# teticio/audio-diffusion

Hardware: NVIDIA H100
Metric: mel-spectrograms/sec (1000-step DDPM, 256x256x1) (higher is better)
Workload: dtype bf16 operands, fp32 accumulate (fp32 master weights, fp64 GroupNorm sums)

## Files before the change

audio_diffusion_b200/_lib.py:

```python
from __future__ import annotations

import ctypes as C
import os

_HERE = os.path.dirname(os.path.abspath(__file__))
LIB_PATH = os.environ.get("B200AD_LIB") or os.path.join(_HERE, "libb200ad.so")

MAX_BLOCKS = 8


class UNetConfigC(C.Structure):
    _fields_ = [
        ("in_channels", C.c_int), ("out_channels", C.c_int), ("layers_per_block", C.c_int), ("num_blocks", C.c_int),
        ("block_out_channels", C.c_int * MAX_BLOCKS), ("down_attn", C.c_int * MAX_BLOCKS),
        ("up_attn", C.c_int * MAX_BLOCKS), ("norm_num_groups", C.c_int), ("norm_eps", C.c_float),
        ("attention_head_dim", C.c_int), ("cross_attention_dim", C.c_int), ("down_cross", C.c_int * MAX_BLOCKS),
        ("up_cross", C.c_int * MAX_BLOCKS),
    ]


class VAEConfigC(C.Structure):
    _fields_ = [
        ("in_channels", C.c_int), ("out_channels", C.c_int), ("latent_channels", C.c_int), ("layers_per_block", C.c_int),
        ("num_blocks", C.c_int), ("block_out_channels", C.c_int * MAX_BLOCKS), ("norm_num_groups", C.c_int),
# ... 26 lines not shown
    "b200ad_unet_param_name": (C.c_char_p, [_VP, _I]),
    "b200ad_unet_param_shape": (_I, [_VP, _I, C.POINTER(C.c_int64)]),
    "b200ad_unet_packed_bytes": (_SZ, [_VP]),
    "b200ad_unet_workspace_bytes": (_SZ, [_VP, _I, _I, _I]),
    "b200ad_unet_set_params": (_I, [_VP, C.POINTER(_VP), _VP, _SZ, _VP]),
    "b200ad_unet_bind_workspace": (_I, [_VP, _VP, _SZ, _I, _I, _I, _VP]),
    "b200ad_unet_forward": (_I, [_VP, _VP, _VP, _VP, _VP]),
    "b200ad_unet_set_encoding": (_I, [_VP, _VP, _I]),
    "b200ad_unet_forward_step": (_I, [_VP, _VP, _VP, _VP, C.POINTER(StepCoefC), _VP, _VP, _VP]),
    "b200ad_unet_forward_step_dev": (_I, [_VP, _VP, _VP, _VP, _VP, _VP, _VP]),
    "b200ad_step_scalars_upload": (_I, [C.POINTER(StepCoefC), C.c_float, _VP, _VP, C.c_int, _VP]),
    "b200ad_unet_profile_step": (_I, [_VP, _VP, _VP, _VP, C.POINTER(StepCoefC), _VP, C.POINTER(C.c_float),
                                      C.POINTER(_I), C.POINTER(C.c_double), _I, _VP]),
    "b200ad_unet_debug_tensor": (_I, [_VP, C.c_char_p, _VP, C.POINTER(_I), _VP]),
    "b200ad_unet_last_launch_count": (_I, [_VP]),
    "b200ad_unet_set_training": (_I, [_VP, _I]),
    "b200ad_unet_grad_floats": (_SZ, [_VP]),
    "b200ad_unet_grad_offset": (_SZ, [_VP, _I]),
    "b200ad_unet_backward_bytes": (_SZ, [_VP]),
    "b200ad_unet_bind_backward": (_I, [_VP, _VP, _SZ, _VP, _VP]),
    "b200ad_unet_backward": (_I, [_VP, _VP, _VP, _I, _VP]),
    "b200ad_unet_backward_launch_count": (_I, [_VP]),
    "b200ad_vae_set_training": (_I, [_VP, _I]),
    "b200ad_vae_grad_floats": (_SZ, [_VP]),
    "b200ad_vae_grad_offset": (_SZ, [_VP, _I]),
    "b200ad_vae_backward_bytes": (_SZ, [_VP]),
    "b200ad_vae_bind_backward": (_I, [_VP, _VP, _SZ, _VP, _VP]),
    "b200ad_vae_decoder_backward": (_I, [_VP, _VP, _VP, _I, _VP]),
    "b200ad_vae_encoder_backward": (_I, [_VP, _VP, _VP, _I, _VP]),
    "b200ad_vae_backward_launch_count": (_I, [_VP]),
# ... 74 lines not shown
```

audio_diffusion_b200/csrc/common.cuh:

```cuda
#pragma once
#include <cuda_bf16.h>
#include <cuda_runtime.h>
#include <stdint.h>
#include <stdio.h>

namespace b200ad {

typedef double stat_t;

struct Geom {
  int N, H, W, Wp, lead, PL;
};
__host__ __device__ inline Geom make_geom(int N, int H, int W) {
  Geom g;
  g.N = N; g.H = H; g.W = W; g.Wp = W + 1; g.lead = g.Wp + 8;
  g.PL = g.lead + H * g.Wp + g.Wp + 8 + 512;
  return g;
}

#ifdef __CUDACC__
__device__ __forceinline__ uint32_t smem_u32(const void* p) {
  return static_cast<uint32_t>(__cvta_generic_to_shared(p));
}
__device__ __forceinline__ void mbar_init(uint32_t bar, uint32_t count) {
// ... 49 lines not shown
__device__ __forceinline__ void bulk_wait_read_all() { asm volatile("cp.async.bulk.wait_group.read 0;" ::: "memory"); }
__device__ __forceinline__ void bulk_wait_all() { asm volatile("cp.async.bulk.wait_group 0;" ::: "memory"); }
__device__ __forceinline__ void named_bar_sync(int id, int nthreads) {
  asm volatile("bar.sync %0, %1;" ::"r"(id), "r"(nthreads) : "memory");
}

__device__ __forceinline__ void tensor_g2s_5d(uint32_t dst_smem, const void* tmap, int c0, int c1, int c2, int c3, int c4,
                                              uint32_t bar) {
  asm volatile(
      "cp.async.bulk.tensor.5d.shared::cluster.global.tile.mbarrier::complete_tx::bytes [%0], [%1, {%2, %3, %4, %5, %6}], [%7];"
      ::"r"(dst_smem), "l"(tmap), "r"(c0), "r"(c1), "r"(c2), "r"(c3), "r"(c4), "r"(bar) : "memory");
}
__device__ __forceinline__ void tensor_s2g_5d(const void* tmap, int c0, int c1, int c2, int c3, int c4, uint32_t src_smem) {
  asm volatile("cp.async.bulk.tensor.5d.global.shared::cta.tile.bulk_group [%0, {%1, %2, %3, %4, %5}], [%6];"
               ::"l"(tmap), "r"(c0), "r"(c1), "r"(c2), "r"(c3), "r"(c4), "r"(src_smem) : "memory");
}

__device__ __forceinline__ void bulk_prefetch_l2(const void* src, uint32_t bytes) {
  asm volatile("cp.async.bulk.prefetch.L2.global [%0], %1;" ::"l"(src), "r"(bytes) : "memory");
}

__device__ __forceinline__ uint64_t gmma_desc(uint32_t saddr, uint32_t lbo_bytes, uint32_t sbo_bytes) {
  uint64_t d = 0;
  d |= (uint64_t)((saddr >> 4) & 0x3FFF);
  d |= (uint64_t)((lbo_bytes >> 4) & 0x3FFF) << 16;
  d |= (uint64_t)((sbo_bytes >> 4) & 0x3FFF) << 32;
  return d;
}
__device__ __forceinline__ void wgmma_fence() { asm volatile("wgmma.fence.sync.aligned;" ::: "memory"); }
__device__ __forceinline__ void wgmma_commit() { asm volatile("wgmma.commit_group.sync.aligned;" ::: "memory"); }
// ... 65 lines not shown
        "+f"(d[24]), "+f"(d[25]), "+f"(d[26]), "+f"(d[27]), "+f"(d[28]), "+f"(d[29]), "+f"(d[30]), "+f"(d[31]),
        "+f"(d[32]), "+f"(d[33]), "+f"(d[34]), "+f"(d[35]), "+f"(d[36]), "+f"(d[37]), "+f"(d[38]), "+f"(d[39]),
        "+f"(d[40]), "+f"(d[41]), "+f"(d[42]), "+f"(d[43]), "+f"(d[44]), "+f"(d[45]), "+f"(d[46]), "+f"(d[47]),
        "+f"(d[48]), "+f"(d[49]), "+f"(d[50]), "+f"(d[51]), "+f"(d[52]), "+f"(d[53]), "+f"(d[54]), "+f"(d[55]),
        "+f"(d[56]), "+f"(d[57]), "+f"(d[58]), "+f"(d[59]), "+f"(d[60]), "+f"(d[61]), "+f"(d[62]), "+f"(d[63]),
        "+f"(d[64]), "+f"(d[65]), "+f"(d[66]), "+f"(d[67]), "+f"(d[68]), "+f"(d[69]), "+f"(d[70]), "+f"(d[71]),
        "+f"(d[72]), "+f"(d[73]), "+f"(d[74]), "+f"(d[75]), "+f"(d[76]), "+f"(d[77]), "+f"(d[78]), "+f"(d[79]),
        "+f"(d[80]), "+f"(d[81]), "+f"(d[82]), "+f"(d[83]), "+f"(d[84]), "+f"(d[85]), "+f"(d[86]), "+f"(d[87]),
        "+f"(d[88]), "+f"(d[89]), "+f"(d[90]), "+f"(d[91]), "+f"(d[92]), "+f"(d[93]), "+f"(d[94]), "+f"(d[95]),
        "+f"(d[96]), "+f"(d[97]), "+f"(d[98]), "+f"(d[99]), "+f"(d[100]), "+f"(d[101]), "+f"(d[102]), "+f"(d[103]),
        "+f"(d[104]), "+f"(d[105]), "+f"(d[106]), "+f"(d[107]), "+f"(d[108]), "+f"(d[109]), "+f"(d[110]), "+f"(d[111]),
        "+f"(d[112]), "+f"(d[113]), "+f"(d[114]), "+f"(d[115]), "+f"(d[116]), "+f"(d[117]), "+f"(d[118]), "+f"(d[119]),
        "+f"(d[120]), "+f"(d[121]), "+f"(d[122]), "+f"(d[123]), "+f"(d[124]), "+f"(d[125]), "+f"(d[126]), "+f"(d[127])
      : "l"(a), "l"(b), "r"(1), "n"(TA), "n"(TB));
}

__device__ __forceinline__ bool elect_one() {
  uint32_t pred;
  asm volatile(
      "{\n\t.reg .pred p;\n\t"
      "elect.sync _|p, 0xffffffff;\n\t"
      "selp.u32 %0, 1, 0, p;\n\t}"
      : "=r"(pred));
  return pred != 0;
}

__device__ __forceinline__ void fence_proxy_async_smem() { asm volatile("fence.proxy.async.shared::cta;" ::: "memory"); }

__device__ __forceinline__ float tanh_approx(float x) {
  float y;
// ... 48 lines not shown
```

audio_diffusion_b200/csrc/conv_tc.cu:

```cuda
#include <cuda.h>
#include <cudaTypedefs.h>

#include <cstdlib>

#include "conv_tc.cuh"

namespace b200ad {

struct alignas(64) ConvMaps {
  CUtensorMap src[CONV_MAXSEG];
  CUtensorMap out;
};

__host__ __device__ __forceinline__ int window_pixels(const ConvParams& p, const ConvSeg& sg, int G) {
  return p.tile2d ? (CONV_TW + sg.hl + sg.hr) * (CONV_TH + sg.ht + sg.hb)
                  : G * CONV_TM + (sg.ht + sg.hb) * p.Wp + sg.hl + sg.hr;
}
__host__ __device__ __forceinline__ int window_pitch(const ConvParams& p, const ConvSeg& sg) {
  return p.tile2d ? CONV_TW + sg.hl + sg.hr : p.Wp;
}

constexpr int CONV_THREADS = 384;
constexpr int CONV_XF_THREADS = 64;
constexpr int CONV_SPLANE = CONV_MAXG * CONV_TM * 16;
constexpr int CONV_STG_WG = 8 * CONV_SPLANE;
constexpr int CONV_STAGING = 2 * CONV_STG_WG;

struct WorkItem {
  int n, ntile, m0, G;
  int r0, c0;
};

__device__ __forceinline__ WorkItem decode_work(const ConvParams& p, int w) {
  WorkItem wi;
  wi.ntile = w % p.ntiles_n;
  const int gidx = w / p.ntiles_n;
  if (p.tile2d) {
    wi.n = gidx / p.groups_per_img;
    const int t = gidx - wi.n * p.groups_per_img, tx = t / p.tiles_y;
    wi.r0 = (t - tx * p.tiles_y) * CONV_TH;
    wi.c0 = tx * CONV_TW;
    wi.m0 = 0;
    wi.G = CONV_MAXG;
    return wi;
  }
  wi.r0 = wi.c0 = 0;
  if (p.pack) {
    wi.n = gidx * p.pack;
    wi.m0 = 0;
    wi.G = min(p.pack, p.N - wi.n);
    return wi;
  }
  wi.n = gidx / p.groups_per_img;
  const int g = gidx - wi.n * p.groups_per_img;
  wi.m0 = g * (CONV_MAXG * CONV_TM);
  const int rem = p.H * p.Wp - wi.m0;
// ... 4 lines not shown
template <bool SILU>
__device__ __forceinline__ uint4 xform_vec(uint4 v, const f32x2_t (&sc)[4], const f32x2_t (&sh)[4]) {
  uint32_t u[4] = {v.x, v.y, v.z, v.w};
#pragma unroll
  for (int e = 0; e < 4; ++e) {
    f32x2_t a = f2_fma(f2_from_bf16x2(u[e]), sc[e], sh[e]);
    if (SILU) {
      const float2 f = f2_unpack(a);
      a = f2_fma(a, f2_pack(tanh_approx(f.x), tanh_approx(f.y)), a);
    }
    u[e] = f2_to_bf16x2(a);
  }
  return make_uint4(u[0], u[1], u[2], u[3]);
}

__global__ void __launch_bounds__(CONV_THREADS, 1) conv_tc_kernel(const __grid_constant__ ConvParams p,
                                                                  const __grid_constant__ ConvMaps maps) {
  constexpr int ASM = CONV_AS_MAX, BSM = CONV_BS_MAX;
  const int AS = p.as;
  const int BS = p.bs;
  extern __shared__ __align__(128) uint8_t smem[];
  const int warp = __shfl_sync(0xffffffffu, (int)(threadIdx.x >> 5), 0);
  const int lane = threadIdx.x & 31;
  const int a_bytes = p.a_stage;

  uint8_t* bring = smem + AS * a_bytes;
  uint8_t* stg = bring + BS * CONV_B_SLOT;
  uint8_t* ctrl = stg + CONV_STAGING;
  uint64_t* bars = reinterpret_cast<uint64_t*>(ctrl);
  const uint32_t smem_base = smem_u32(smem);
// ... 28 lines not shown
    for (int w = blockIdx.x; w < p.total_work; w += gridDim.x) {
      const WorkItem wi = decode_work(p, w);
      for (int s = 0; s < p.nseg; ++s) {
        const ConvSeg& sg = p.seg[s];
        const uint32_t row_bytes = (uint32_t)window_pixels(p, sg, wi.G) * 16u;
        for (int ks = 0; ks < sg.ksteps; ++ks) {
          const uint32_t full = bar_fullA + 8 * stage;
          if (lane == 0) {
            mbar_wait(bar_emptyA + 8 * stage, phase ^ 1);
            mbar_arrive_expect_tx(full, 2u * row_bytes);
          }
          __syncwarp();
          const long long plane = (long long)(2 * ks + (lane & 1)) * p.PL;
          if (p.tile2d) {
            if (lane == 0)
              tensor_g2s_5d(smem_base + stage * a_bytes, &maps.src[s], 0, wi.c0 - sg.hl, wi.r0 - sg.ht, 2 * ks, wi.n, full);
          } else if (!p.pack) {
            const int pix0 = p.lead + wi.m0 - sg.ht * p.Wp - sg.hl;
            if (lane < 2)
              bulk_g2s(smem_base + stage * a_bytes + (uint32_t)lane * row_bytes,
                       sg.src + (long long)wi.n * sg.img_stride + (plane + pix0) * 8, row_bytes, full);
          } else {
            const int g = lane >> 1, lead_px = sg.ht * p.Wp + sg.hl, trail_px = sg.hb * p.Wp + sg.hr;
            const int cnt = CONV_TM + (g == 0 ? lead_px : 0) + (g == wi.G - 1 ? trail_px : 0);
            const int doff = (g == 0) ? 0 : lead_px + g * CONV_TM;
            const int pix0 = p.lead - (g == 0 ? lead_px : 0);
            if (g < wi.G && lane < 2 * CONV_MAXG)
              bulk_g2s(smem_base + stage * a_bytes + (uint32_t)(lane & 1) * row_bytes + (uint32_t)doff * 16u,
                       sg.src + (long long)(wi.n + g) * sg.img_stride + (plane + pix0) * 8, (uint32_t)cnt * 16u, full);
          }
          if (++stage == AS) { stage = 0; phase ^= 1; }
// ... 53 lines not shown
      for (int s = 0, ks = 0; s < p.nseg;) {
        const ConvSeg& sg = p.seg[s];
        const uint32_t xlbo = (uint32_t)window_pixels(p, sg, wi.G) * 16u;
        const uint32_t xsbo = p.tile2d ? (uint32_t)window_pitch(p, sg) * 16u : 128u;
        const int ntaps = sg.ntaps;
        mbar_wait(bar_readyA + 8 * sa, pa);
        const uint32_t abase = smem_base + sa * a_bytes;
        for (int t0 = 0; t0 < ntaps; t0 += CONV_BT) {
          mbar_wait(bar_fullB + 8 * sb, pb);
          const uint32_t bbase = bring_base + sb * CONV_B_SLOT + (uint32_t)(cw * 1024);
          const int nt = min(CONV_BT, ntaps - t0);
          wgmma_fence();
          for (int t = 0; t < nt; ++t) {
            const uint64_t wdesc = gmma_desc(bbase + (uint32_t)t * CONV_B_TAP, (CONV_NT / 8) * 128, 128);
            const uint64_t xdesc = gmma_desc(abase + (uint32_t)sg.aoff[t0 + t] * 16u, xlbo, xsbo);
            if (wi.G == 2) wgmma_m64n256k16<0, 0>(acc, wdesc, xdesc);
            else           wgmma_m64n128k16<0, 0>(acc, wdesc, xdesc);
          }
          wgmma_commit();
          wgmma_wait<1>();
          release();
          pend_b = sb;
          pend_a = (t0 + CONV_BT >= ntaps) ? sa : -1;
          if (++sb == BS) { sb = 0; pb ^= 1; }
        }
        if (++sa == AS) { sa = 0; pa ^= 1; }
        if (++ks == sg.ksteps) { ks = 0; ++s; }
      }
      wgmma_wait<0>();
      release();

      if (issuer) bulk_wait_read_all();
// ... 48 lines not shown
                  const int c = wi.ntile * CONV_NT + cw * 64 + wq * 16 + 8 * h + (lane >> 2);
                  stat_t* sdst = p.stats + ((long long)n * (p.cout >> 2) + (c >> 2)) * 2;
                  atomicAdd(sdst, (stat_t)s1);
                  atomicAdd(sdst + 1, (stat_t)s2);
                }
                ssum[h] = 0.f;
                ssq[h] = 0.f;
              }
            }
          }
        }
      }
      if (p.tile2d) {
        fence_proxy_async_smem();
        named_bar_sync(1 + cw, 128);
        if (tid == 0 && !(p.dbg & 2)) {
          tensor_s2g_5d(&maps.out, 0, wi.c0, wi.r0, wi.ntile * 16 + cw * 8, wi.n, stg_w);
          bulk_commit();
        }
      } else if (!p.up2) {
        fence_proxy_async_smem();
        named_bar_sync(1 + cw, 128);
        const int g = tid >> 3, pl = tid & 7;
        if (issuer && g < wi.G && !(p.dbg & 2)) {
          const int n = p.pack ? wi.n + g : wi.n;
          bulk_s2g(p.out + (long long)n * out_img_stride + (long long)(wi.ntile * 16 + cw * 8 + pl) * og.PL * 8 +
                       (long long)(p.lead + (p.pack ? 0 : wi.m0 + CONV_TM * g)) * 8,
                   stg_w + (uint32_t)(pl * CONV_SPLANE + g * CONV_TM * 16), (uint32_t)CONV_TM * 16u);
          bulk_commit();
        }
      } else {
        named_bar_sync(1 + cw, 128);
// ... 151 lines not shown
        int n = i / Ct, c = i - n * Ct;
        for (; i < total; i += CONV_THREADS) {
          const int gi = n * f.groups + (int)(((float)c + 0.5f) * inv_cpg);
          const float sc = __ldg(f.gamma + c) * grstd[gi];
          f.ss[i] = make_float2(sc, __ldg(f.beta + c) - gmean[gi] * sc);
          n += dn;
          c += dc;
          if (c >= Ct) { c -= Ct; ++n; }
        }
      }
      if (threadIdx.x == 0) *f.counter = 0u;
    }
  }
}

static cudaError_t encode_pf8_map(CUtensorMap* m, const __nv_bfloat16* base, const ConvParams& p, int planes,
                                  long long img_stride, int bw, int bh, int bplanes) {
  static PFN_cuTensorMapEncodeTiled_v12000 encode = nullptr;
  if (!encode) {
    void* fn = nullptr;
    cudaDriverEntryPointQueryResult q;
    cudaError_t e = cudaGetDriverEntryPointByVersion("cuTensorMapEncodeTiled", &fn, 12000, cudaEnableDefault, &q);
    if (e != cudaSuccess) return e;
    if (q != cudaDriverEntryPointSuccess || !fn) return cudaErrorNotSupported;
    encode = reinterpret_cast<PFN_cuTensorMapEncodeTiled_v12000>(fn);
  }
  const cuuint64_t dim[5] = {8, (cuuint64_t)p.W, (cuuint64_t)p.H, (cuuint64_t)planes, (cuuint64_t)p.N};
  const cuuint64_t stride[4] = {16, (cuuint64_t)p.Wp * 16, (cuuint64_t)p.PL * 16, (cuuint64_t)img_stride * 2};
  const cuuint32_t box[5] = {8, (cuuint32_t)bw, (cuuint32_t)bh, (cuuint32_t)bplanes, 1};
  const cuuint32_t estride[5] = {1, 1, 1, 1, 1};
  const CUresult r = encode(m, CU_TENSOR_MAP_DATA_TYPE_BFLOAT16, 5, (void*)(base + (long long)p.lead * 8), dim, stride, box,
                            estride, CU_TENSOR_MAP_INTERLEAVE_NONE, CU_TENSOR_MAP_SWIZZLE_NONE, CU_TENSOR_MAP_L2_PROMOTION_L2_256B,
                            CU_TENSOR_MAP_FLOAT_OOB_FILL_NONE);
  return r == CUDA_SUCCESS ? cudaSuccess : cudaErrorInvalidValue;
}

cudaError_t launch_conv_tc(const ConvParams& p_in, int num_sms, cudaStream_t stream) {
  const char* dbg_env = getenv("B200AD_CONV_DBG");
  const int dbg = dbg_env ? atoi(dbg_env) : 0;
  if (p_in.nseg < 1 || p_in.nseg > CONV_MAXSEG) return cudaErrorInvalidValue;
  ConvParams p = p_in;
  p.dbg = dbg;
  for (int s = 0; s < p.nseg; ++s) {
    ConvSeg& sg = p.seg[s];
    if (sg.ntaps > CONV_MAXTAPS || sg.ksteps < 1) return cudaErrorInvalidValue;
    if (sg.wtile_stride == 0) sg.wtile_stride = (long long)sg.ksteps * sg.ntaps * (CONV_B_TAP / 2);
    sg.ht = sg.hb = sg.hl = sg.hr = 0;
    for (int t = 0; t < sg.ntaps; ++t) {
      sg.ht |= sg.dh[t] < 0; sg.hb |= sg.dh[t] > 0;
      sg.hl |= sg.dw[t] < 0; sg.hr |= sg.dw[t] > 0;
    }
  }
  p.groups_per_img = (p.H * p.Wp + CONV_MAXG * CONV_TM - 1) / (CONV_MAXG * CONV_TM);
  p.ntiles_n = p.cout / CONV_NT;
  p.total_work = p.N * p.groups_per_img * p.ntiles_n;
  p.pack = 0;
  int fits = 1;
  for (int s = 0; s < p.nseg; ++s) {
    const ConvSeg& sg = p.seg[s];
    if (p.H * p.Wp + sg.hb * p.Wp + sg.hr > CONV_TM || sg.ht * p.Wp + sg.hl > CONV_TM) fits = 0;
  }
  if (fits) {
    int best = 1;
    long long best_cost = -1;
    for (int g = 1; g <= CONV_MAXG; g *= 2) {
      const long long items = (long long)((p.N + g - 1) / g) * p.ntiles_n;
      const long long cost = ((items + num_sms - 1) / num_sms) * g;
      if (best_cost < 0 || cost <= best_cost) { best_cost = cost; best = g; }
    }
    p.pack = best;
    p.total_work = ((p.N + best - 1) / best) * p.ntiles_n;
  }
  const int tiles_img = (p.H * p.Wp + CONV_TM - 1) / CONV_TM;
  const int max_g = p.pack ? p.pack : (tiles_img < CONV_MAXG ? tiles_img : CONV_MAXG);
  p.tile2d = 0;
  if (!p.pack && !p.up2 && !(dbg & 4096) && p.W % CONV_TW == 0 && p.H % CONV_TH == 0) {
    ConvParams q = p;
    q.tile2d = 1;
    long long flat = 0, tiled = 0;
    for (int s = 0; s < p.nseg; ++s) {
      flat += window_pixels(p, p.seg[s], max_g);
      tiled += window_pixels(q, p.seg[s], max_g);
    }
    if (tiled < flat) {
      p.tile2d = 1;
      p.tiles_y = p.H / CONV_TH;
      p.groups_per_img = (p.W / CONV_TW) * p.tiles_y;
      p.total_work = p.N * p.groups_per_img * p.ntiles_n;
    }
  }
  int a_stage = 0;
  for (int s = 0; s < p.nseg; ++s) {
    const ConvSeg& sg = p.seg[s];
    const int npix = window_pixels(p, sg, max_g), pitch = window_pitch(p, sg);
    a_stage = npix * 32 > a_stage ? npix * 32 : a_stage;
    if (sg.ntaps > CONV_MAXTAPS || sg.ntaps > CONV_BT * (CONV_BS - 1) || npix > 0x3FFF) return cudaErrorInvalidValue;
    for (int t = 0; t < sg.ntaps; ++t) p.seg[s].aoff[t] = (sg.dh[t] + sg.ht) * pitch + sg.dw[t] + sg.hl;
  }
  p.a_stage = (a_stage + 255) & ~255;
  ConvMaps maps{};
  if (p.tile2d) {
    for (int s = 0; s < p.nseg; ++s) {
      const ConvSeg& sg = p.seg[s];
      cudaError_t e = encode_pf8_map(&maps.src[s], sg.src, p, 2 * sg.ksteps, sg.img_stride, CONV_TW + sg.hl + sg.hr,
                                     CONV_TH + sg.ht + sg.hb, 2);
      if (e != cudaSuccess) return e;
    }
    cudaError_t e = encode_pf8_map(&maps.out, p.out, p, p.cout / 8, (long long)(p.cout / 8) * p.PL * 8, CONV_TW, CONV_TH, 8);
    if (e != cudaSuccess) return e;
  }
  p.as = CONV_AS;
  p.bs = CONV_BS;
  auto rings_fit = [&](int as, int bs) {
    return (size_t)as * p.a_stage + (size_t)bs * CONV_B_SLOT + CONV_STAGING + 2048 <= (size_t)CONV_SMEM_MAX;
  };
  while (p.as < 6 && rings_fit(p.as + 1, p.bs)) ++p.as;
  while (p.bs < CONV_BS_MAX && rings_fit(p.as, p.bs + 1)) ++p.bs;
  while (p.as < CONV_AS_MAX && rings_fit(p.as + 1, p.bs)) ++p.as;
  const size_t smem = (size_t)p.as * p.a_stage + (size_t)p.bs * CONV_B_SLOT + CONV_STAGING + 1024;
  if (smem > (size_t)CONV_SMEM_MAX) return cudaErrorInvalidValue;
  const int grid = p.total_work < num_sms ? p.total_work : num_sms;
  if (grid <= 0) return cudaSuccess;
  static size_t attr = 0;
  if (smem > attr) {
    cudaError_t e = cudaFuncSetAttribute(conv_tc_kernel, cudaFuncAttributeMaxDynamicSharedMemorySize, (int)smem);
    if (e != cudaSuccess) return e;
    attr = smem;
  }
  cudaLaunchConfig_t cfg = {};
  cfg.gridDim = dim3((unsigned)grid);
  cfg.blockDim = dim3(CONV_THREADS);
  cfg.dynamicSmemBytes = smem;
  cfg.stream = stream;
  cudaLaunchAttribute at[1];
  at[0].id = cudaLaunchAttributeProgrammaticStreamSerialization;
  at[0].val.programmaticStreamSerializationAllowed = 1;
  cfg.attrs = at;
  cfg.numAttrs = 1;
  return cudaLaunchKernelEx(&cfg, conv_tc_kernel, p, maps);
}

__global__ void pack_identity_kernel(int channels, __nv_bfloat16* __restrict__ dst, long long nvec) {
  const long long id = (long long)blockIdx.x * blockDim.x + threadIdx.x;
  if (id >= nvec) return;
  const int r = (int)(id & 7), n8 = (int)((id >> 3) & 15), k8 = (int)((id >> 7) & 1);
  const long long rest = id >> 8;
  const int ksteps = channels / 16;
  const int ks = (int)(rest % ksteps), ntile = (int)(rest / ksteps);
  const int co = ntile * 128 + n8 * 8 + r;
  const int ci0 = ks * 16 + k8 * 8;
  uint32_t o[4];
#pragma unroll
  for (int e = 0; e < 4; ++e) o[e] = pack_bf16x2(co == ci0 + 2 * e ? 1.f : 0.f, co == ci0 + 2 * e + 1 ? 1.f : 0.f);
  reinterpret_cast<uint4*>(dst)[id] = make_uint4(o[0], o[1], o[2], o[3]);
// ... 9 lines not shown
```

audio_diffusion_b200/csrc/conv_tc.cuh:

```cuda
#pragma once
#include "common.cuh"

namespace b200ad {

constexpr int CONV_NT = 128;
constexpr int CONV_TM = 128;
constexpr int CONV_MAXG = 2;
constexpr int CONV_TW = 8;
constexpr int CONV_TH = CONV_MAXG * CONV_TM / CONV_TW;
constexpr int CONV_MAXSEG = 4;
constexpr int CONV_MAXTAPS = 9;
constexpr int CONV_B_TAP = 16 * CONV_NT * 2;
constexpr int CONV_SMEM_MAX = 227 * 1024;

constexpr int CONV_BT = 3;
constexpr int CONV_B_SLOT = CONV_BT * CONV_B_TAP;
constexpr int CONV_AS_MAX = 8;
constexpr int CONV_AS = 3;
constexpr int CONV_BS = 5;
constexpr int CONV_BS_MAX = 10;

struct ConvSeg {
  const __nv_bfloat16* src;
  const __nv_bfloat16* wpack;
// ... 15 lines not shown
  int C[2];
  const float* gamma;
  const float* beta;
  float2* ss;
  unsigned* counter;
  int groups, HW;
  float eps;
};

struct ConvParams {
  ConvSeg seg[CONV_MAXSEG];
  int nseg;
  int N, H, W, Wp, lead, PL;
  int a_stage;
  int tile2d;
  int tiles_y;
  int groups_per_img;
  int ntiles_n;
  int total_work;
  int pack;
  int as, bs;
  int cout;
  __nv_bfloat16* out;
  const float* bias;
  const float* temb;
  int temb_stride;
  stat_t* stats;
  int up2, oy, ox;
  ConvGnFin fin;
  int dbg;
};

cudaError_t launch_conv_tc(const ConvParams& p, int num_sms, cudaStream_t stream);

cudaError_t launch_pack_identity(int channels, __nv_bfloat16* dst, cudaStream_t s);

}
```

audio_diffusion_b200/csrc/unet.cu:

```cuda
#include "unet.cuh"

namespace b200ad {

thread_local char g_err[512] = "";
int set_err(const char* fmt, ...) {
  va_list ap;
  va_start(ap, fmt);
  vsnprintf(g_err, sizeof(g_err), fmt, ap);
  va_end(ap);
  return -1;
}

}

using namespace b200ad;


namespace b200ad {

static std::vector<Block> unet_blocks(const b200ad_unet_config& c) {
  const int nb = c.num_blocks, D = c.block_out_channels[0] * 4, X = c.cross_attention_dim;
  const int* boc = c.block_out_channels;
  std::vector<Block> bl;
  add_block(bl, BK_UNET_HEAD, "", c.in_channels, boc[0], "").temb = D;
// ... 192 lines not shown
      double k = 0;
      for (int s = 0; s < p.nseg; ++s) {
        bool ident = false;
        for (const auto& kv : h->ident_off)
          if ((const uint8_t*)p.seg[s].wpack == h->packed + kv.second) ident = true;
        if (!ident) k += (double)(p.up2 ? 9 : p.seg[s].ntaps) * p.seg[s].ksteps * 16;
      }
      fl = 2.0 * p.N * p.H * p.W * p.cout * k;
    }
    op_flops[i] = fl;
  }
  for (auto& e : ev) cudaEventDestroy(e);
  return nops;
}

extern "C" int b200ad_unet_set_encoding(b200ad_unet* h, const float* enc, int S) {
  if (!h->cfg.cross_attention_dim) return set_err("set_encoding: this U-Net is unconditional");
  if (S < 1) return set_err("set_encoding: empty encoder sequence");
  h->enc = enc;
  h->enc_S = S;
  return 0;
}

extern "C" int b200ad_unet_forward(b200ad_unet* h, const float* x, const float* t, float* eps_out, void* stream) {
  RunArgs a;
  a.in = x; a.t = t; a.out = eps_out;
  return run_plan(h, a, (cudaStream_t)stream);
}
extern "C" int b200ad_unet_forward_step(b200ad_unet* h, const float* x, const float* t, const float* z,
                                        const b200ad_step_coef* coef, float* x_out, float* eps_out, void* stream) {
// ... 30 lines not shown
```

include/b200ad.h:

```cpp
#ifndef B200AD_H
#define B200AD_H
#include <stddef.h>
#include <stdint.h>

#ifdef __cplusplus
extern "C" {
#endif

#define B200AD_MAX_BLOCKS 8

const char* b200ad_last_error(void);
int b200ad_version(void);

typedef struct {
  int in_channels, out_channels;
  int layers_per_block;
  int num_blocks;
  int block_out_channels[B200AD_MAX_BLOCKS];
  int down_attn[B200AD_MAX_BLOCKS];
  int up_attn[B200AD_MAX_BLOCKS];
  int norm_num_groups;
  float norm_eps;
  int attention_head_dim;
  int cross_attention_dim;
// ... 29 lines not shown
int b200ad_unet_forward_step(b200ad_unet* h, const float* x, const float* t, const float* z,
                             const b200ad_step_coef* coef, float* x_out, float* eps_out, void* stream);

int b200ad_unet_forward_step_dev(b200ad_unet* h, const float* x, const float* t, const float* z,
                                 const b200ad_step_coef* coef_dev, float* x_out, void* stream);
int b200ad_step_scalars_upload(const b200ad_step_coef* coef, float t, b200ad_step_coef* coef_dev, float* t_dev, int n,
                               void* stream);

int b200ad_unet_debug_tensor(b200ad_unet* h, const char* name, float* dst, int* dims, void* stream);

int b200ad_unet_profile_step(b200ad_unet* h, const float* x, const float* t, const float* z,
                             const b200ad_step_coef* coef, float* x_out, float* op_ms, int* op_kind,
                             double* op_flops, int max_ops, void* stream);

int b200ad_unet_last_launch_count(const b200ad_unet* h);

int b200ad_unet_set_training(b200ad_unet* h, int on);
size_t b200ad_unet_grad_floats(b200ad_unet* h);
size_t b200ad_unet_grad_offset(b200ad_unet* h, int i);
size_t b200ad_unet_backward_bytes(b200ad_unet* h);
int b200ad_unet_bind_backward(b200ad_unet* h, void* arena, size_t bytes, float* grads, void* stream);
int b200ad_unet_backward(b200ad_unet* h, const float* x, const float* g_eps, int accumulate, void* stream);
int b200ad_unet_backward_launch_count(const b200ad_unet* h);

typedef struct {
  int in_channels, out_channels;
  int latent_channels;
  int layers_per_block;
  int num_blocks;
  int block_out_channels[B200AD_MAX_BLOCKS];
// ... 86 lines not shown
```

Baseline: 0.8489.

## Add 16x16 square 2D conv tiles with cost-based tile shape selection

Generalizes the 2D-tiled implicit-GEMM conv from a fixed 8x32 window to selectable 8x32 or 16x16 tiles. A planner scores each shape by padded work, item count and halo-window pixels per k-step. A templated SQUARE kernel path issues paired m64n128 wgmma instructions and per-row TMA stores, and the TMA maps move to a 4D layout. Square tiles are also enabled for upsample-fused convs, which reduces halo reloads but adds more store instructions and more planner complexity; a plan-inspection API is exported as well.

```diff
diff --git a/audio_diffusion_b200/_lib.py b/audio_diffusion_b200/_lib.py
--- a/audio_diffusion_b200/_lib.py
+++ b/audio_diffusion_b200/_lib.py
@@ -64,6 +64,7 @@
                                       C.POINTER(_I), C.POINTER(C.c_double), _I, _VP]),
     "b200ad_unet_debug_tensor": (_I, [_VP, C.c_char_p, _VP, C.POINTER(_I), _VP]),
     "b200ad_unet_last_launch_count": (_I, [_VP]),
+    "b200ad_unet_conv_plan": (_I, [_VP, _I, _I, _I, _I, C.POINTER(_I), _I]),
     "b200ad_unet_set_training": (_I, [_VP, _I]),
     "b200ad_unet_grad_floats": (_SZ, [_VP]),
     "b200ad_unet_grad_offset": (_SZ, [_VP, _I]),
diff --git a/audio_diffusion_b200/csrc/common.cuh b/audio_diffusion_b200/csrc/common.cuh
--- a/audio_diffusion_b200/csrc/common.cuh
+++ b/audio_diffusion_b200/csrc/common.cuh
@@ -87,6 +87,16 @@
 __device__ __forceinline__ void tensor_s2g_5d(const void* tmap, int c0, int c1, int c2, int c3, int c4, uint32_t src_smem) {
   asm volatile("cp.async.bulk.tensor.5d.global.shared::cta.tile.bulk_group [%0, {%1, %2, %3, %4, %5}], [%6];"
                ::"l"(tmap), "r"(c0), "r"(c1), "r"(c2), "r"(c3), "r"(c4), "r"(src_smem) : "memory");
+}
+
+__device__ __forceinline__ void tensor_g2s_4d(uint32_t dst_smem, const void* tmap, int c0, int c1, int c2, int c3, uint32_t bar) {
+  asm volatile(
+      "cp.async.bulk.tensor.4d.shared::cluster.global.tile.mbarrier::complete_tx::bytes [%0], [%1, {%2, %3, %4, %5}], [%6];"
+      ::"r"(dst_smem), "l"(tmap), "r"(c0), "r"(c1), "r"(c2), "r"(c3), "r"(bar) : "memory");
+}
+__device__ __forceinline__ void tensor_s2g_4d(const void* tmap, int c0, int c1, int c2, int c3, uint32_t src_smem) {
+  asm volatile("cp.async.bulk.tensor.4d.global.shared::cta.tile.bulk_group [%0, {%1, %2, %3, %4}], [%5];"
+               ::"l"(tmap), "r"(c0), "r"(c1), "r"(c2), "r"(c3), "r"(src_smem) : "memory");
 }
 
 __device__ __forceinline__ void bulk_prefetch_l2(const void* src, uint32_t bytes) {
@@ -182,6 +192,39 @@
         "+f"(d[120]), "+f"(d[121]), "+f"(d[122]), "+f"(d[123]), "+f"(d[124]), "+f"(d[125]), "+f"(d[126]), "+f"(d[127])
       : "l"(a), "l"(b), "r"(1), "n"(TA), "n"(TB));
 }
+__device__ __forceinline__ void wgmma_m64n128k16_x2(float* d, uint64_t a, uint64_t b0, uint64_t b1) {
+  asm volatile(
+      "{\n\t.reg .pred p;\n\tsetp.ne.b32 p, %131, 0;\n\t"
+      "wgmma.mma_async.sync.aligned.m64n128k16.f32.bf16.bf16 {"
+      "%0, %1, %2, %3, %4, %5, %6, %7, %8, %9, %10, %11, %12, %13, %14, %15, "
+      "%16, %17, %18, %19, %20, %21, %22, %23, %24, %25, %26, %27, %28, %29, %30, %31, "
+      "%32, %33, %34, %35, %36, %37, %38, %39, %40, %41, %42, %43, %44, %45, %46, %47, "
+      "%48, %49, %50, %51, %52, %53, %54, %55, %56, %57, %58, %59, %60, %61, %62, %63"
+      "}, %128, %129, p, 1, 1, 0, 0;\n\t"
+      "wgmma.mma_async.sync.aligned.m64n128k16.f32.bf16.bf16 {"
+      "%64, %65, %66, %67, %68, %69, %70, %71, %72, %73, %74, %75, %76, %77, %78, %79, "
+      "%80, %81, %82, %83, %84, %85, %86, %87, %88, %89, %90, %91, %92, %93, %94, %95, "
+      "%96, %97, %98, %99, %100, %101, %102, %103, %104, %105, %106, %107, %108, %109, %110, %111, "
+      "%112, %113, %114, %115, %116, %117, %118, %119, %120, %121, %122, %123, %124, %125, %126, %127"
+      "}, %128, %130, p, 1, 1, 0, 0;\n\t}"
+      : "+f"(d[0]), "+f"(d[1]), "+f"(d[2]), "+f"(d[3]), "+f"(d[4]), "+f"(d[5]), "+f"(d[6]), "+f"(d[7]),
+        "+f"(d[8]), "+f"(d[9]), "+f"(d[10]), "+f"(d[11]), "+f"(d[12]), "+f"(d[13]), "+f"(d[14]), "+f"(d[15]),
+        "+f"(d[16]), "+f"(d[17]), "+f"(d[18]), "+f"(d[19]), "+f"(d[20]), "+f"(d[21]), "+f"(d[22]), "+f"(d[23]),
+        "+f"(d[24]), "+f"(d[25]), "+f"(d[26]), "+f"(d[27]), "+f"(d[28]), "+f"(d[29]), "+f"(d[30]), "+f"(d[31]),
+        "+f"(d[32]), "+f"(d[33]), "+f"(d[34]), "+f"(d[35]), "+f"(d[36]), "+f"(d[37]), "+f"(d[38]), "+f"(d[39]),
+        "+f"(d[40]), "+f"(d[41]), "+f"(d[42]), "+f"(d[43]), "+f"(d[44]), "+f"(d[45]), "+f"(d[46]), "+f"(d[47]),
+        "+f"(d[48]), "+f"(d[49]), "+f"(d[50]), "+f"(d[51]), "+f"(d[52]), "+f"(d[53]), "+f"(d[54]), "+f"(d[55]),
+        "+f"(d[56]), "+f"(d[57]), "+f"(d[58]), "+f"(d[59]), "+f"(d[60]), "+f"(d[61]), "+f"(d[62]), "+f"(d[63]),
+        "+f"(d[64]), "+f"(d[65]), "+f"(d[66]), "+f"(d[67]), "+f"(d[68]), "+f"(d[69]), "+f"(d[70]), "+f"(d[71]),
+        "+f"(d[72]), "+f"(d[73]), "+f"(d[74]), "+f"(d[75]), "+f"(d[76]), "+f"(d[77]), "+f"(d[78]), "+f"(d[79]),
+        "+f"(d[80]), "+f"(d[81]), "+f"(d[82]), "+f"(d[83]), "+f"(d[84]), "+f"(d[85]), "+f"(d[86]), "+f"(d[87]),
+        "+f"(d[88]), "+f"(d[89]), "+f"(d[90]), "+f"(d[91]), "+f"(d[92]), "+f"(d[93]), "+f"(d[94]), "+f"(d[95]),
+        "+f"(d[96]), "+f"(d[97]), "+f"(d[98]), "+f"(d[99]), "+f"(d[100]), "+f"(d[101]), "+f"(d[102]), "+f"(d[103]),
+        "+f"(d[104]), "+f"(d[105]), "+f"(d[106]), "+f"(d[107]), "+f"(d[108]), "+f"(d[109]), "+f"(d[110]), "+f"(d[111]),
+        "+f"(d[112]), "+f"(d[113]), "+f"(d[114]), "+f"(d[115]), "+f"(d[116]), "+f"(d[117]), "+f"(d[118]), "+f"(d[119]),
+        "+f"(d[120]), "+f"(d[121]), "+f"(d[122]), "+f"(d[123]), "+f"(d[124]), "+f"(d[125]), "+f"(d[126]), "+f"(d[127])
+      : "l"(a), "l"(b0), "l"(b1), "r"(1));
+}
 
 __device__ __forceinline__ bool elect_one() {
   uint32_t pred;
diff --git a/audio_diffusion_b200/csrc/conv_tc.cu b/audio_diffusion_b200/csrc/conv_tc.cu
--- a/audio_diffusion_b200/csrc/conv_tc.cu
+++ b/audio_diffusion_b200/csrc/conv_tc.cu
@@ -13,11 +13,11 @@
 };
 
 __host__ __device__ __forceinline__ int window_pixels(const ConvParams& p, const ConvSeg& sg, int G) {
-  return p.tile2d ? (CONV_TW + sg.hl + sg.hr) * (CONV_TH + sg.ht + sg.hb)
+  return p.tile2d ? (p.tw + sg.hl + sg.hr) * (p.th + sg.ht + sg.hb)
                   : G * CONV_TM + (sg.ht + sg.hb) * p.Wp + sg.hl + sg.hr;
 }
 __host__ __device__ __forceinline__ int window_pitch(const ConvParams& p, const ConvSeg& sg) {
-  return p.tile2d ? CONV_TW + sg.hl + sg.hr : p.Wp;
+  return p.tile2d ? p.tw + sg.hl + sg.hr : p.Wp;
 }
 
 constexpr int CONV_THREADS = 384;
@@ -25,6 +25,9 @@
 constexpr int CONV_SPLANE = CONV_MAXG * CONV_TM * 16;
 constexpr int CONV_STG_WG = 8 * CONV_SPLANE;
 constexpr int CONV_STAGING = 2 * CONV_STG_WG;
+static size_t conv_smem_bytes(const ConvParams& p) {
+  return (size_t)p.as * p.a_stage + (size_t)p.bs * CONV_B_SLOT + CONV_STAGING + 1024;
+}
 
 struct WorkItem {
   int n, ntile, m0, G;
@@ -38,8 +41,8 @@
   if (p.tile2d) {
     wi.n = gidx / p.groups_per_img;
     const int t = gidx - wi.n * p.groups_per_img, tx = t / p.tiles_y;
-    wi.r0 = (t - tx * p.tiles_y) * CONV_TH;
-    wi.c0 = tx * CONV_TW;
+    wi.r0 = (t - tx * p.tiles_y) * p.th;
+    wi.c0 = tx * p.tw;
     wi.m0 = 0;
     wi.G = CONV_MAXG;
     return wi;
@@ -74,6 +77,7 @@
   return make_uint4(u[0], u[1], u[2], u[3]);
 }
 
+template <bool SQUARE>
 __global__ void __launch_bounds__(CONV_THREADS, 1) conv_tc_kernel(const __grid_constant__ ConvParams p,
                                                                   const __grid_constant__ ConvMaps maps) {
   constexpr int ASM = CONV_AS_MAX, BSM = CONV_BS_MAX;
@@ -132,7 +136,7 @@
           const long long plane = (long long)(2 * ks + (lane & 1)) * p.PL;
           if (p.tile2d) {
             if (lane == 0)
-              tensor_g2s_5d(smem_base + stage * a_bytes, &maps.src[s], 0, wi.c0 - sg.hl, wi.r0 - sg.ht, 2 * ks, wi.n, full);
+              tensor_g2s_4d(smem_base + stage * a_bytes, &maps.src[s], 8 * (wi.c0 - sg.hl), wi.r0 - sg.ht, 2 * ks, wi.n, full);
           } else if (!p.pack) {
             const int pix0 = p.lead + wi.m0 - sg.ht * p.Wp - sg.hl;
             if (lane < 2)
@@ -216,8 +220,13 @@
           for (int t = 0; t < nt; ++t) {
             const uint64_t wdesc = gmma_desc(bbase + (uint32_t)t * CONV_B_TAP, (CONV_NT / 8) * 128, 128);
             const uint64_t xdesc = gmma_desc(abase + (uint32_t)sg.aoff[t0 + t] * 16u, xlbo, xsbo);
-            if (wi.G == 2) wgmma_m64n256k16<0, 0>(acc, wdesc, xdesc);
-            else           wgmma_m64n128k16<0, 0>(acc, wdesc, xdesc);
+            if constexpr (SQUARE) {
+              wgmma_m64n128k16_x2(acc, wdesc, xdesc, xdesc + (128u >> 4));
+            } else if (wi.G == 2) {
+              wgmma_m64n256k16<0, 0>(acc, wdesc, xdesc);
+            } else {
+              wgmma_m64n128k16<0, 0>(acc, wdesc, xdesc);
+            }
           }
           wgmma_commit();
           wgmma_wait<1>();
@@ -296,8 +305,17 @@
       if (p.tile2d) {
         fence_proxy_async_smem();
         named_bar_sync(1 + cw, 128);
-        if (tid == 0 && !(p.dbg & 2)) {
-          tensor_s2g_5d(&maps.out, 0, wi.c0, wi.r0, wi.ntile * 16 + cw * 8, wi.n, stg_w);
+        if (SQUARE) {
+          const int g = tid >> 3, pl = tid & 7;
+          if (issuer && !(p.dbg & 2)) {
+            const uint32_t src = stg_w + (uint32_t)(pl * CONV_SPLANE + g * CONV_TM * 16);
+            const int c = wi.c0 + 8 * g, plane = wi.ntile * 16 + cw * 8 + pl;
+            if (p.up2) tensor_s2g_5d(&maps.out, 0, c, wi.r0, plane, wi.n, src);
+            else       tensor_s2g_4d(&maps.out, 8 * c, wi.r0, plane, wi.n, src);
+            bulk_commit();
+          }
+        } else if (tid == 0 && !(p.dbg & 2)) {
+          tensor_s2g_4d(&maps.out, 8 * wi.c0, wi.r0, wi.ntile * 16 + cw * 8, wi.n, stg_w);
           bulk_commit();
         }
       } else if (!p.up2) {
@@ -479,8 +497,8 @@
   }
 }
 
-static cudaError_t encode_pf8_map(CUtensorMap* m, const __nv_bfloat16* base, const ConvParams& p, int planes,
-                                  long long img_stride, int bw, int bh, int bplanes) {
+static cudaError_t encode_pf8_map(CUtensorMap* m, const __nv_bfloat16* base, const ConvParams& p, int cs, int rs, long long pl,
+                                  int planes, long long img_stride, int bw, int bh, int bplanes) {
   static PFN_cuTensorMapEncodeTiled_v12000 encode = nullptr;
   if (!encode) {
     void* fn = nullptr;
@@ -490,22 +508,31 @@
     if (q != cudaDriverEntryPointSuccess || !fn) return cudaErrorNotSupported;
     encode = reinterpret_cast<PFN_cuTensorMapEncodeTiled_v12000>(fn);
   }
-  const cuuint64_t dim[5] = {8, (cuuint64_t)p.W, (cuuint64_t)p.H, (cuuint64_t)planes, (cuuint64_t)p.N};
-  const cuuint64_t stride[4] = {16, (cuuint64_t)p.Wp * 16, (cuuint64_t)p.PL * 16, (cuuint64_t)img_stride * 2};
-  const cuuint32_t box[5] = {8, (cuuint32_t)bw, (cuuint32_t)bh, (cuuint32_t)bplanes, 1};
   const cuuint32_t estride[5] = {1, 1, 1, 1, 1};
-  const CUresult r = encode(m, CU_TENSOR_MAP_DATA_TYPE_BFLOAT16, 5, (void*)(base + (long long)p.lead * 8), dim, stride, box,
-                            estride, CU_TENSOR_MAP_INTERLEAVE_NONE, CU_TENSOR_MAP_SWIZZLE_NONE, CU_TENSOR_MAP_L2_PROMOTION_L2_256B,
-                            CU_TENSOR_MAP_FLOAT_OOB_FILL_NONE);
+  CUresult r;
+  if (cs == 1) {
+    const cuuint64_t dim[4] = {(cuuint64_t)p.W * 8, (cuuint64_t)p.H, (cuuint64_t)planes, (cuuint64_t)p.N};
+    const cuuint64_t stride[3] = {(cuuint64_t)rs * 16, (cuuint64_t)pl * 16, (cuuint64_t)img_stride * 2};
+    const cuuint32_t box[4] = {(cuuint32_t)bw * 8, (cuuint32_t)bh, (cuuint32_t)bplanes, 1};
+    r = encode(m, CU_TENSOR_MAP_DATA_TYPE_BFLOAT16, 4, (void*)base, dim, stride, box, estride, CU_TENSOR_MAP_INTERLEAVE_NONE,
+               CU_TENSOR_MAP_SWIZZLE_NONE, CU_TENSOR_MAP_L2_PROMOTION_L2_256B, CU_TENSOR_MAP_FLOAT_OOB_FILL_NONE);
+  } else {
+    const cuuint64_t dim[5] = {8, (cuuint64_t)p.W, (cuuint64_t)p.H, (cuuint64_t)planes, (cuuint64_t)p.N};
+    const cuuint64_t stride[4] = {(cuuint64_t)cs * 16, (cuuint64_t)rs * 16, (cuuint64_t)pl * 16, (cuuint64_t)img_stride * 2};
+    const cuuint32_t box[5] = {8, (cuuint32_t)bw, (cuuint32_t)bh, (cuuint32_t)bplanes, 1};
+    r = encode(m, CU_TENSOR_MAP_DATA_TYPE_BFLOAT16, 5, (void*)base, dim, stride, box, estride, CU_TENSOR_MAP_INTERLEAVE_NONE,
+               CU_TENSOR_MAP_SWIZZLE_NONE, CU_TENSOR_MAP_L2_PROMOTION_L2_256B, CU_TENSOR_MAP_FLOAT_OOB_FILL_NONE);
+  }
   return r == CUDA_SUCCESS ? cudaSuccess : cudaErrorInvalidValue;
 }
 
-cudaError_t launch_conv_tc(const ConvParams& p_in, int num_sms, cudaStream_t stream) {
+int conv_dbg_env() {
   const char* dbg_env = getenv("B200AD_CONV_DBG");
-  const int dbg = dbg_env ? atoi(dbg_env) : 0;
-  if (p_in.nseg < 1 || p_in.nseg > CONV_MAXSEG) return cudaErrorInvalidValue;
-  ConvParams p = p_in;
-  p.dbg = dbg;
+  return dbg_env ? atoi(dbg_env) : 0;
+}
+
+cudaError_t plan_conv_tc(ConvParams& p, int num_sms) {
+  if (p.nseg < 1 || p.nseg > CONV_MAXSEG) return cudaErrorInvalidValue;
   for (int s = 0; s < p.nseg; ++s) {
     ConvSeg& sg = p.seg[s];
     if (sg.ntaps > CONV_MAXTAPS || sg.ksteps < 1) return cudaErrorInvalidValue;
@@ -516,6 +543,9 @@
       sg.hl |= sg.dw[t] < 0; sg.hr |= sg.dw[t] > 0;
     }
   }
+  p.tile2d = 0;
+  p.tw = p.th = 0;
+  p.tiles_y = 0;
   p.groups_per_img = (p.H * p.Wp + CONV_MAXG * CONV_TM - 1) / (CONV_MAXG * CONV_TM);
   p.ntiles_n = p.cout / CONV_NT;
   p.total_work = p.N * p.groups_per_img * p.ntiles_n;
@@ -538,19 +568,32 @@
   }
   const int tiles_img = (p.H * p.Wp + CONV_TM - 1) / CONV_TM;
   const int max_g = p.pack ? p.pack : (tiles_img < CONV_MAXG ? tiles_img : CONV_MAXG);
-  p.tile2d = 0;
-  if (!p.pack && !p.up2 && !(dbg & 4096) && p.W % CONV_TW == 0 && p.H % CONV_TH == 0) {
-    ConvParams q = p;
-    q.tile2d = 1;
-    long long flat = 0, tiled = 0;
-    for (int s = 0; s < p.nseg; ++s) {
-      flat += window_pixels(p, p.seg[s], max_g);
-      tiled += window_pixels(q, p.seg[s], max_g);
-    }
-    if (tiled < flat) {
-      p.tile2d = 1;
-      p.tiles_y = p.H / CONV_TH;
-      p.groups_per_img = (p.W / CONV_TW) * p.tiles_y;
+  if (!p.pack && !(p.dbg & 4096)) {
+    auto window_cost = [&](const ConvParams& q, int G) {
+      long long c = 0;
+      for (int s = 0; s < q.nseg; ++s) c += (long long)window_pixels(q, q.seg[s], G) * q.seg[s].ksteps;
+      return c;
+    };
+    long long best[3] = {(long long)tiles_img * CONV_TM, p.groups_per_img, 0};
+    for (int i = 0; i < p.groups_per_img; ++i) best[2] += window_cost(p, min(CONV_MAXG, tiles_img - CONV_MAXG * i));
+    const int shapes[2][2] = {{8, 32}, {16, 16}};
+    for (const auto& sh : shapes) {
+      const int tw = sh[0], th = sh[1];
+      if (p.W % tw || p.H % th) continue;
+      if (tw == 16 && p.H >= 64 && p.H % 32 == 0 && p.W % 8 == 0) continue;
+      if (tw == 8 && p.up2) continue;
+      ConvParams q = p;
+      q.tile2d = 1; q.tw = tw; q.th = th;
+      const long long items = (long long)(p.W / tw) * (p.H / th);
+      const long long c[3] = {items * CONV_MAXG * CONV_TM, items, items * window_cost(q, CONV_MAXG)};
+      if (c[0] < best[0] || (c[0] == best[0] && (c[1] < best[1] || (c[1] == best[1] && c[2] < best[2])))) {
+        best[0] = c[0]; best[1] = c[1]; best[2] = c[2];
+        p.tile2d = 1; p.tw = tw; p.th = th;
+      }
+    }
+    if (p.tile2d) {
+      p.tiles_y = p.H / p.th;
+      p.groups_per_img = (p.W / p.tw) * p.tiles_y;
       p.total_work = p.N * p.groups_per_img * p.ntiles_n;
     }
   }
@@ -563,17 +606,6 @@
     for (int t = 0; t < sg.ntaps; ++t) p.seg[s].aoff[t] = (sg.dh[t] + sg.ht) * pitch + sg.dw[t] + sg.hl;
   }
   p.a_stage = (a_stage + 255) & ~255;
-  ConvMaps maps{};
-  if (p.tile2d) {
-    for (int s = 0; s < p.nseg; ++s) {
-      const ConvSeg& sg = p.seg[s];
-      cudaError_t e = encode_pf8_map(&maps.src[s], sg.src, p, 2 * sg.ksteps, sg.img_stride, CONV_TW + sg.hl + sg.hr,
-                                     CONV_TH + sg.ht + sg.hb, 2);
-      if (e != cudaSuccess) return e;
-    }
-    cudaError_t e = encode_pf8_map(&maps.out, p.out, p, p.cout / 8, (long long)(p.cout / 8) * p.PL * 8, CONV_TW, CONV_TH, 8);
-    if (e != cudaSuccess) return e;
-  }
   p.as = CONV_AS;
   p.bs = CONV_BS;
   auto rings_fit = [&](int as, int bs) {
@@ -582,15 +614,44 @@
   while (p.as < 6 && rings_fit(p.as + 1, p.bs)) ++p.as;
   while (p.bs < CONV_BS_MAX && rings_fit(p.as, p.bs + 1)) ++p.bs;
   while (p.as < CONV_AS_MAX && rings_fit(p.as + 1, p.bs)) ++p.as;
-  const size_t smem = (size_t)p.as * p.a_stage + (size_t)p.bs * CONV_B_SLOT + CONV_STAGING + 1024;
-  if (smem > (size_t)CONV_SMEM_MAX) return cudaErrorInvalidValue;
+  if (conv_smem_bytes(p) > (size_t)CONV_SMEM_MAX) return cudaErrorInvalidValue;
+  return cudaSuccess;
+}
+
+cudaError_t launch_conv_tc(const ConvParams& p_in, int num_sms, cudaStream_t stream) {
+  ConvParams p = p_in;
+  p.dbg = conv_dbg_env();
+  if (cudaError_t e = plan_conv_tc(p, num_sms)) return e;
+  ConvMaps maps{};
+  if (p.tile2d) {
+    for (int s = 0; s < p.nseg; ++s) {
+      const ConvSeg& sg = p.seg[s];
+      cudaError_t e = encode_pf8_map(&maps.src[s], sg.src + (long long)p.lead * 8, p, 1, p.Wp, p.PL, 2 * sg.ksteps,
+                                     sg.img_stride, p.tw + sg.hl + sg.hr, p.th + sg.ht + sg.hb, 2);
+      if (e != cudaSuccess) return e;
+    }
+    const int bh = p.th, bplanes = p.tw == 16 ? 1 : 8;
+    cudaError_t e;
+    if (p.up2) {
+      const Geom og = make_geom(p.N, 2 * p.H, 2 * p.W);
+      e = encode_pf8_map(&maps.out, p.out + (long long)(og.lead + p.oy * og.Wp + p.ox) * 8, p, 2, 2 * og.Wp, og.PL,
+                         p.cout / 8, (long long)(p.cout / 8) * og.PL * 8, 8, bh, bplanes);
+    } else {
+      e = encode_pf8_map(&maps.out, p.out + (long long)p.lead * 8, p, 1, p.Wp, p.PL, p.cout / 8,
+                         (long long)(p.cout / 8) * p.PL * 8, 8, bh, bplanes);
+    }
+    if (e != cudaSuccess) return e;
+  }
+  const size_t smem = conv_smem_bytes(p);
   const int grid = p.total_work < num_sms ? p.total_work : num_sms;
   if (grid <= 0) return cudaSuccess;
-  static size_t attr = 0;
-  if (smem > attr) {
-    cudaError_t e = cudaFuncSetAttribute(conv_tc_kernel, cudaFuncAttributeMaxDynamicSharedMemorySize, (int)smem);
+  const bool square = p.tile2d && p.tw == 16;
+  void (*kernel)(ConvParams, ConvMaps) = square ? conv_tc_kernel<true> : conv_tc_kernel<false>;
+  static size_t attr[2] = {0, 0};
+  if (smem > attr[square]) {
+    cudaError_t e = cudaFuncSetAttribute(kernel, cudaFuncAttributeMaxDynamicSharedMemorySize, (int)smem);
     if (e != cudaSuccess) return e;
-    attr = smem;
+    attr[square] = smem;
   }
   cudaLaunchConfig_t cfg = {};
   cfg.gridDim = dim3((unsigned)grid);
@@ -602,7 +663,7 @@
   at[0].val.programmaticStreamSerializationAllowed = 1;
   cfg.attrs = at;
   cfg.numAttrs = 1;
-  return cudaLaunchKernelEx(&cfg, conv_tc_kernel, p, maps);
+  return cudaLaunchKernelEx(&cfg, kernel, p, maps);
 }
 
 __global__ void pack_identity_kernel(int channels, __nv_bfloat16* __restrict__ dst, long long nvec) {
diff --git a/audio_diffusion_b200/csrc/conv_tc.cuh b/audio_diffusion_b200/csrc/conv_tc.cuh
--- a/audio_diffusion_b200/csrc/conv_tc.cuh
+++ b/audio_diffusion_b200/csrc/conv_tc.cuh
@@ -6,8 +6,6 @@
 constexpr int CONV_NT = 128;
 constexpr int CONV_TM = 128;
 constexpr int CONV_MAXG = 2;
-constexpr int CONV_TW = 8;
-constexpr int CONV_TH = CONV_MAXG * CONV_TM / CONV_TW;
 constexpr int CONV_MAXSEG = 4;
 constexpr int CONV_MAXTAPS = 9;
 constexpr int CONV_B_TAP = 16 * CONV_NT * 2;
@@ -53,6 +51,7 @@
   int N, H, W, Wp, lead, PL;
   int a_stage;
   int tile2d;
+  int tw, th;
   int tiles_y;
   int groups_per_img;
   int ntiles_n;
@@ -70,6 +69,8 @@
   int dbg;
 };
 
+cudaError_t plan_conv_tc(ConvParams& p, int num_sms);
+int conv_dbg_env();
 cudaError_t launch_conv_tc(const ConvParams& p, int num_sms, cudaStream_t stream);
 
 cudaError_t launch_pack_identity(int channels, __nv_bfloat16* dst, cudaStream_t s);
diff --git a/audio_diffusion_b200/csrc/unet.cu b/audio_diffusion_b200/csrc/unet.cu
--- a/audio_diffusion_b200/csrc/unet.cu
+++ b/audio_diffusion_b200/csrc/unet.cu
@@ -230,6 +230,24 @@
   return nops;
 }
 
+extern "C" int b200ad_unet_conv_plan(const b200ad_unet* h, int N, int H, int W, int num_sms, int* rows, int max_rows) {
+  const Plan pl = build_plan(h, nullptr, N, H, W);
+  const int dbg = conv_dbg_env();
+  int n = 0;
+  for (const Op& op : pl.lists[0].ops) {
+    if (op.kind != OP_CONV) continue;
+    if (n >= max_rows) return set_err("conv_plan: more than %d conv launches", max_rows);
+    ConvParams p = op.conv;
+    p.dbg = dbg;
+    if (plan_conv_tc(p, num_sms) != cudaSuccess) return set_err("conv_plan: launch %d cannot be planned", n);
+    const int row[B200AD_CONV_PLAN_COLS] = {p.H, p.W, p.seg[0].ksteps * 16, p.cout, p.nseg, p.up2,
+                                             p.pack, p.tw, p.th, p.total_work, p.as, p.bs};
+    for (int c = 0; c < B200AD_CONV_PLAN_COLS; ++c) rows[n * B200AD_CONV_PLAN_COLS + c] = row[c];
+    ++n;
+  }
+  return n;
+}
+
 extern "C" int b200ad_unet_set_encoding(b200ad_unet* h, const float* enc, int S) {
   if (!h->cfg.cross_attention_dim) return set_err("set_encoding: this U-Net is unconditional");
   if (S < 1) return set_err("set_encoding: empty encoder sequence");
diff --git a/include/b200ad.h b/include/b200ad.h
--- a/include/b200ad.h
+++ b/include/b200ad.h
@@ -67,6 +67,9 @@
                              double* op_flops, int max_ops, void* stream);
 
 int b200ad_unet_last_launch_count(const b200ad_unet* h);
+
+#define B200AD_CONV_PLAN_COLS 12
+int b200ad_unet_conv_plan(const b200ad_unet* h, int N, int H, int W, int num_sms, int* rows, int max_rows);
 
 int b200ad_unet_set_training(b200ad_unet* h, int on);
 size_t b200ad_unet_grad_floats(b200ad_unet* h);
```

Result: faster. 0.9253, median of 6 (+9.0%).
